# RVC-Project/obs-rvc

Hardware: AMD Instinct MI355X
Metric: audio frames/sec (10 ms hops of new input, 160 ms chunks @16 kHz) (higher is better)
Workload: dtype f32; 1 GPU; BASELINE configs[1]: 1 stream(s)/GPU, ContentVec v2-768 + RMVPE + NSF-HiFiGAN v2-48k, retrieval off, preset full; streams_per_gpu=1, streams_total=1, hip_graph=False

## Files before the change

obs_rvc_amd/csrc/conv_tile.hip.h:

```cpp
#pragma once
#include "igemm.hip.h"

namespace rvc {

#define COMMA_ ,
#ifndef RVC_CT_DBG
#define RVC_CT_DBG 0
#endif
template <int ACT, int MF, int NF>
__device__ __forceinline__ void conv_tile_store(const IgemmP &p, const PhaseD &ph, const float *resb, float *yb, const ColOut (&cols)[NF], int m_base, const f32x4 (&acc)[MF][NF])
{
    const float slope = p.slope, scale = p.scale;
    const long long cs = p.y_cs, rcs = p.res_cs;
#pragma unroll
    for (int mf = 0; mf < MF; mf++) {
        const int m0 = m_base + mf * 16;
        float bias_r[4];
#pragma unroll
        for (int r = 0; r < 4; r++) bias_r[r] = (p.bias && m0 + r < p.M) ? p.bias[ph.bias_off + m0 + r] : 0.f;
#pragma unroll
        for (int nf = 0; nf < NF; nf++) {
            if (cols[nf].yo < 0) continue;
            float rr[4] = {0.f, 0.f, 0.f, 0.f}, yo[4] = {0.f, 0.f, 0.f, 0.f};
            float *yc = yb + cols[nf].yo + (long long)(m0 + ph.y_c0) * cs;
            if (resb) {
                const float *rp = resb + cols[nf].ro + (long long)(p.res_nogroup ? m0 : m0 + ph.y_c0) * rcs;
#pragma unroll
                for (int r = 0; r < 4; r++) if (m0 + r < p.M) rr[r] = rp[r * rcs];
            }
            if (p.accumulate) {
#pragma unroll
                for (int r = 0; r < 4; r++) if (m0 + r < p.M) yo[r] = yc[r * cs];
            }
#pragma unroll
            for (int r = 0; r < 4; r++)
                if (m0 + r < p.M) yc[r * cs] = epi2_value<ACT>(acc[mf][nf][r], bias_r[r], rr[r], yo[r], slope, scale);
        }
    }
}

template <int WM, int WN, int MF, int NF, int KS>
__global__ __launch_bounds__(64 * WM * WN * KS) __attribute__((amdgpu_waves_per_eu(2))) void conv_tile_kernel(IgemmP p)
{
    static_assert(KS == 1 || KS == 2, "one or two K shares");
    constexpr int WPS = WM * WN, NT = 64 * WPS * KS;
    constexpr int BM = WM * MF * 16, BN = WN * NF * 16;
    constexpr int DA = MF == 1 ? 8 : 6;
    extern __shared__ __attribute__((aligned(16))) int s_mem[];
    const int item = p.items[2 * blockIdx.x];
    if (item < 0) return;
    RVC_KP(0);
    const int phase = item & 0xff, tm = (item >> 8) & 0xff, tn = item >> 16;
    const int b = p.items[2 * blockIdx.x + 1];
    const PhaseD ph = p.nphase == 1 ? p.ph0 : p.ph[phase];
    const int nchunks = ph.nchunks;
    const int lane = threadIdx.x & 63;
    const int wave = __builtin_amdgcn_readfirstlane((int)(threadIdx.x >> 6));
    const int kh = wave / WPS, w4 = wave % WPS;
    const int wm = w4 / WN, wn = w4 % WN;
    const int li = lane & 15, kq = lane >> 4;
    const int cin = ph.t_cin, rt = ph.t_rs, kw = ph.t_tab & 0xff, dil = ph.t_tab >> 8;
    const int rl = BN + (kw - 1) * dil;
    const int cs = cin + 8;
    const int G = cin >> 4;
    float *tmp = reinterpret_cast<float *>(s_mem);
    const int tmp_n = (cin * rt + 63) & ~63;
    float *fin = tmp + (tmp_n > WPS * MF * NF * 256 ? tmp_n : WPS * MF * NF * 256);
    {
        const float *xb = p.x + (long long)b * p.x_bs + ph.x_off;
        const int n0 = tn * BN + ph.t_dmin;
        const int total = cin * rt;
        const float inv_rt = 1.0f / (float)rt;
        for (int q = wave; q * 64 < total; q += WPS * KS) {
            const int e = q * 64 + lane;
            int row = (int)(((float)e + 0.5f) * inv_rt);
            const int col = e - row * rt;
            row = row < cin ? row : cin - 1;
            int gc = n0 + col;
            gc = gc < p.x_lo ? p.x_lo : (gc > p.x_lim ? p.x_lim : gc);
            __builtin_amdgcn_global_load_lds(xb + (long long)row * p.x_ld + gc, (__attribute__((address_space(3))) void *)(tmp + q * 64), 4, 0, 0);
        }
    }
    RVC_KP(1);
    const float *wrow[MF];
    const int mtiles = (p.M + 15) >> 4;
#pragma unroll
    for (int mf = 0; mf < MF; mf++) {
        int mt = (tm * WM + wm) * MF + mf;
        mt = mt < mtiles ? mt : mtiles - 1;
        wrow[mf] = p.w + ph.w_off + (long long)mt * nchunks * 256;
    }
    const int nloc = (nchunks - kh + KS - 1) / KS;
    const unsigned lane16 = (unsigned)lane * 16u;
    const float *wnext[MF];
#pragma unroll
    for (int mf = 0; mf < MF; mf++) wnext[mf] = wrow[mf] + (long long)(kh + DA * KS) * 256;
    f32x4 a_st[DA][MF];
#pragma unroll
    for (int s = 0; s < DA; s++) {
        const int cc = kh + (s < nloc ? s : nloc - 1) * KS;
#pragma unroll
        for (int mf = 0; mf < MF; mf++) a_st[s][mf] = *reinterpret_cast<const f32x4 *>(wrow[mf] + cc * 256 + lane * 4);
    }
    f32x4 acc[MF][NF];
#pragma unroll
    for (int mf = 0; mf < MF; mf++)
#pragma unroll
        for (int nf = 0; nf < NF; nf++) acc[mf][nf] = (f32x4){0.f, 0.f, 0.f, 0.f};
    const float pre_slope = p.pre_slope;
    RVC_KP(11);
    __syncthreads();
    {
        const int total = cin * rl;
        const float inv_cin = 1.0f / (float)cin;
        for (int e = threadIdx.x; e < total; e += NT) {
            const int col = (int)(((float)e + 0.5f) * inv_cin), ci = e - col * cin;
            const float v = tmp[ci * rt + col];
            fin[col * cs + ci] = fmaxf(v, v * pre_slope);
        }
    }
    __syncthreads();
    RVC_KP(2);
    const float *bl = fin + (wn * NF * 16 + li) * cs + kq * 4;
    const int last = nloc - 1;
    int g_b = 0, off_b = 0;
    const int wrap_b = dil * cs - 16 * G;
#define RVC_CT_ADV1() { g_b++; off_b += 16; if (g_b == G) { g_b = 0; off_b += wrap_b; } }
#define RVC_CT_ADV() { g_b += KS; off_b += 16 * KS; if (g_b >= G) { g_b -= G; off_b += wrap_b; } }
    if (kh) RVC_CT_ADV1()
    f32x4 bcur[NF];
#pragma unroll
    for (int nf = 0; nf < NF; nf++) bcur[nf] = *reinterpret_cast<const f32x4 *>(bl + off_b + nf * 16 * cs);
    RVC_CT_ADV()
    constexpr int T_ = MF * NF * 4;
#define RVC_CT_STEP(S, CC)                                                                              \
    {                                                                                                  \
        const int cc_ = (CC);                                                                          \
        const int ob_ = cc_ < last ? off_b : 0;                  \
        f32x4 bnx_[NF];                                                                                \
        _Pragma("unroll") for (int t = 0; t < T_; t++) {                                               \
            const int j = t / (NF * MF), nf = (t / MF) % NF, mf = t % MF;                              \
            if (!(RVC_CT_DBG & 8)) acc[mf][nf] = __builtin_amdgcn_mfma_f32_16x16x4f32(a_st[S][mf][j], bcur[nf][j], acc[mf][nf], 0, 0, 0); \
            else acc[mf][nf][0] += a_st[S][mf][j] * bcur[nf][j];                                       \
                                     \
            _Pragma("unroll") for (int r = t * NF / T_; r < (t + 1) * NF / T_; r++) {                  \
                if (!(RVC_CT_DBG & 2)) bnx_[r] = *reinterpret_cast<const f32x4 *>(bl + ob_ + r * 16 * cs); else bnx_[r] = bcur[r]; \
            }                                                                                          \
            __builtin_amdgcn_sched_barrier(0);                                                         \
        }                                                                                              \
         \
        if (!(RVC_CT_DBG & 1)) {                                                                       \
            _Pragma("unroll") for (int mf = 0; mf < MF; mf++) a_st[S][mf] = *reinterpret_cast<const f32x4 *>(reinterpret_cast<const char *>(wnext[mf]) + lane16); \
        }                                                                                              \
        __builtin_amdgcn_sched_barrier(0);                                                             \
        RVC_CT_ADV()                                                                                   \
        _Pragma("unroll") for (int mf = 0; mf < MF; mf++) wnext[mf] += KS * 256;       \
        _Pragma("unroll") for (int nf = 0; nf < NF; nf++) bcur[nf] = bnx_[nf];                         \
    }
    int c = 0;
    for (; c + DA <= nloc; c += DA) {
#pragma unroll
        for (int s = 0; s < DA; s++) RVC_CT_STEP(s, c + s)
    }
#pragma unroll
    for (int s = 0; s < DA; s++)
        if (c + s < nloc) RVC_CT_STEP(s, c + s)
#undef RVC_CT_STEP
#undef RVC_CT_ADV
#undef RVC_CT_ADV1
    RVC_KP(3);
    if (KS == 2) {
        f32x4 *red = reinterpret_cast<f32x4 *>(tmp) + (w4 * MF * NF) * 64 + lane;
        if (kh) {
#pragma unroll
            for (int mf = 0; mf < MF; mf++)
#pragma unroll
                for (int nf = 0; nf < NF; nf++) red[(mf * NF + nf) * 64] = acc[mf][nf];
        }
        __syncthreads();
        if (kh) return;
#pragma unroll
        for (int mf = 0; mf < MF; mf++)
#pragma unroll
            for (int nf = 0; nf < NF; nf++) { const f32x4 o = red[(mf * NF + nf) * 64]; acc[mf][nf][0] += o[0]; acc[mf][nf][1] += o[1]; acc[mf][nf][2] += o[2]; acc[mf][nf][3] += o[3]; }
    }
    const float *resb = p.res ? p.res + (long long)b * p.res_bs : nullptr;
    float *yb = p.y + (long long)b * p.y_bs + ph.y_off;
    const int act_sel = ph.act_p1 ? ph.act_p1 - 1 : p.act;
    ColOut cols[NF];
#pragma unroll
    for (int nf = 0; nf < NF; nf++) cols[nf] = col_locate(p, ph, tn * BN + (wn * NF + nf) * 16 + li);
    RVC_ACT_DISPATCH_SEL(act_sel, conv_tile_store<A_ COMMA_ MF COMMA_ NF>(p, ph, resb, yb, cols, ((tm * WM + wm) * MF) * 16 + kq * 4, acc);)
    RVC_KP(6);
}
#undef COMMA_

}
```

obs_rvc_amd/csrc/debug.hip:

```cpp
#include "engine_int.h"
#include "../../include/rvc_mi355x_debug.h"
#include <deque>

namespace {

struct DebugGeo {
    float *base = nullptr; long long g[8] = {0, 0, 0, 0, 0, 0, 0, 1};
    bool live() const { return base && g[0] > 0; }
    void upload(const float *h) const { if (live()) HIPCHK(hipMemcpy(base, h, (size_t)g[0] * 4, hipMemcpyHostToDevice)); }
    void download(float *h) const { if (live()) HIPCHK(hipMemcpy(h, base, (size_t)g[0] * 4, hipMemcpyDeviceToHost)); }
};
DebugGeo debug_geo1(const T1 &t)
{
    DebugGeo q; const size_t gd = t1_guard(t.ld);
    q.base = t.p - gd - t.halo; q.g[0] = (long long)t.B * t.bs + 2 * (long long)gd; q.g[1] = (long long)gd + t.halo; q.g[2] = t.C; q.g[3] = t.T; q.g[4] = t.ld; q.g[5] = t.bs; q.g[6] = t.ld;
    return q;
}
DebugGeo debug_geo2(const T2 &t)
{
    DebugGeo q; const size_t gd = t2_guard(t.ld);
    q.base = t.p - gd - t.ld - 1; q.g[0] = (long long)t.B * t.bs + 2 * (long long)gd; q.g[1] = (long long)gd + t.ld + 1; q.g[2] = t.C; q.g[3] = t.W; q.g[4] = t.ld; q.g[5] = t.bs; q.g[6] = t.cs; q.g[7] = t.H;
    return q;
}
DebugGeo debug_geo_flat(float *p, long long n, int C, int T) { DebugGeo q; q.base = p; q.g[0] = n; q.g[1] = 0; q.g[2] = C; q.g[3] = T; q.g[4] = T; q.g[5] = (long long)C * T; q.g[6] = T; return q; }
// ... 9 lines not shown
        try { for (auto &o : pl.ops.v) o(e->stream); } catch (...) { end_failed_capture(e->stream); throw; }
        HIPCHK(hipStreamEndCapture(e->stream, &g));
        const hipError_t ie = hipGraphInstantiate(&ge, g, nullptr, nullptr, 0);
        (void)hipGraphDestroy(g);
        HIPCHK(ie);
        hipError_t le = hipSuccess;
        for (int r = 0; r < reps && le == hipSuccess; r++) le = hipGraphLaunch(ge, e->stream);
        const hipError_t se = hipStreamSynchronize(e->stream);
        (void)hipGraphExecDestroy(ge);
        HIPCHK(le); HIPCHK(se);
    } else {
        for (int r = 0; r < reps; r++) for (auto &o : pl.ops.v) o(e->stream);
        HIPCHK(hipStreamSynchronize(e->stream));
    }
    HIPCHK(hipGetLastError());
}

struct DebugWeights {
    std::deque<ConvW> convs; std::vector<float *> raw;
    DebugWeights() = default;
    DebugWeights(const DebugWeights &) = delete;
    ConvW &conv(ConvW c) { convs.push_back(std::move(c)); return convs.back(); }
    float *dev(float *p) { raw.push_back(p); return p; }
    ~DebugWeights() { for (ConvW &c : convs) free_conv(c); for (float *p : raw) wfree(p); }
};

void fill_weights(std::vector<float> &w) { for (size_t i = 0; i < w.size(); i++) w[i] = (float)((i * 2654435761u) % 1000) / 1000.0f - 0.5f; }
void fill_input(std::vector<float> &x) { for (size_t i = 0; i < x.size(); i++) x[i] = (float)(((i * 40503u) ^ (i >> 3)) % 2001) / 1000.0f - 1.0f; }

}

extern "C" {

int rvc_debug_stamps(rvc_engine *e, char *buf, size_t cap)
{
    if (!e || !e->last_plan || !e->last_plan->d_stamps) return 0;
    Plan &pl = *e->last_plan;
    std::vector<unsigned long long> h(pl.stamp_names.size());
    if (hipMemcpy(h.data(), pl.d_stamps, h.size() * 8, hipMemcpyDeviceToHost) != hipSuccess) return 0;
    unsigned long long t0 = ~0ull; for (auto v : h) t0 = std::min(t0, v);
    std::string out;
    for (size_t i = 0; i < h.size(); i++) { char ln[96]; snprintf(ln, sizeof ln, "%s %.2f\n", pl.stamp_names[i].c_str(), (double)(h[i] - t0) / 100.0); out += ln; }
    if (out.size() + 1 > cap) return -1;
    memcpy(buf, out.c_str(), out.size() + 1);
    return (int)h.size();
}

#ifdef RVC_TUNING
double rvc_debug_conv_bench(rvc_engine *e, int M, int Cin, int KW, int dil, int N, int iters, int pre_act, int streams, int act)
{
    double us = -1.0;
    (void)guarded(e, [&]() {
        std::vector<float> w((size_t)M * Cin * KW), bias(M, 0.1f);
        fill_weights(w);
        const int Bb = streams > 0 ? streams : 1;
        Plan pl; pl.B = Bb;
        DebugWeights wts;
        ConvW &cw = wts.conv(prep_conv(w.data(), bias.data(), M, Cin, KW, 1));
        const int pad = (KW - 1) * dil / 2;
        T1 x = make_t1(pl.arena, Bb, Cin, N, (pad + 3) / 4 * 4), y = make_t1(pl.arena, Bb, M, N, 0);
        std::vector<float> hx((size_t)Cin * x.ld, 0.25f);
        for (int b = 0; b < Bb; b++) HIPCHK(hipMemcpy(x.p + (long long)b * x.bs - x.halo, hx.data(), hx.size() * 4, hipMemcpyHostToDevice));
        ConvOpts o; if (pre_act) { o.pre_act = ACT_LRELU; o.pre_slope = 0.1f; }
        o.act = act;
        add_conv1d(pl, cw, x, y, 1, pad, dil, o);
        run_ops(e, pl, 3, false);
        hipEvent_t a, b; HIPCHK(hipEventCreate(&a)); HIPCHK(hipEventCreate(&b));
        HIPCHK(hipEventRecord(a, e->stream));
        for (int i = 0; i < iters; i++) for (auto &op : pl.ops.v) op(e->stream);
        HIPCHK(hipEventRecord(b, e->stream));
        HIPCHK(hipStreamSynchronize(e->stream));
        float ms; HIPCHK(hipEventElapsedTime(&ms, a, b));
        us = ms * 1e3 / iters;
        (void)hipEventDestroy(a); (void)hipEventDestroy(b);
        return RVC_OK;
    });
    return us;
}

int rvc_debug_conv_probe(rvc_engine *e, int M, int Cin, int KW, int dil, int N, unsigned long long *out, size_t cap_waves, double *event_us, int *waves_per_wg)
{
    int nw = -1;
    (void)guarded(e, [&]() {
        std::vector<float> w((size_t)M * Cin * KW), bias(M, 0.1f);
        fill_weights(w);
        Plan pl; pl.B = 1;
        DebugWeights wts;
        ConvW &cw = wts.conv(prep_conv(w.data(), bias.data(), M, Cin, KW, 1));
        const int pad = (KW - 1) * dil / 2;
        T1 x = make_t1(pl.arena, 1, Cin, N, (pad + 3) / 4 * 4), y = make_t1(pl.arena, 1, M, N, 0);
        std::vector<float> hx((size_t)Cin * x.ld, 0.25f);
        HIPCHK(hipMemcpy(x.p - x.halo, hx.data(), hx.size() * 4, hipMemcpyHostToDevice));
        const size_t pbytes = (size_t)1 << 24;
        unsigned long long *d_probe = (unsigned long long *)pl.arena.alloc(pbytes);
        ConvOpts o; if (const char *a = tune_env("RVC_BENCH_ACT")) o.act = atoi(a);
        {
            struct Probing { Probing(unsigned long long *p) { g_kprobe = p; } ~Probing() { g_kprobe = nullptr; } } probing(d_probe);
            add_conv1d(pl, cw, x, y, 1, pad, dil, o);
        }
        run_ops(e, pl, 5, false);
        HIPCHK(hipMemset(d_probe, 0, pbytes));
        pl.profile = true; pl.prof_used = 0;
        run_ops(e, pl, 1, false);
        float t = 0.f; HIPCHK(hipEventElapsedTime(&t, pl.prof[0].a, pl.prof[0].b));
        if (event_us) *event_us = t * 1e3;
        nw = g_last_wgs * g_last_waves;
        if (waves_per_wg) *waves_per_wg = g_last_waves;
        if ((size_t)nw <= cap_waves && (size_t)nw * 128 <= pbytes) HIPCHK(hipMemcpy(out, d_probe, (size_t)nw * 128, hipMemcpyDeviceToHost));
        else nw = -2;
        return RVC_OK;
    });
    return nw;
}
#endif

double rvc_debug_ln_fold_check(rvc_engine *e, int M, int K, int N, float offset)
{
    double worst = -1.0;
    (void)guarded(e, [&]() {
        if (K % 16 != 0) throw ShapeError("K must be a multiple of 16");
        auto rnd = [](size_t i, unsigned salt) { return (float)((((i + 1) * 2654435761u) ^ (salt * 40503u) ^ (i >> 5)) % 2001) / 1000.0f - 1.0f; };
        std::vector<float> w1((size_t)M * K), b1(M), w2((size_t)K * M), b2(K), g(K), beta(K), hx((size_t)K * N), hz((size_t)M * N);
        for (size_t i = 0; i < w1.size(); i++) w1[i] = 0.5f * rnd(i, 1);
        for (size_t i = 0; i < w2.size(); i++) w2[i] = 0.5f * rnd(i, 2);
        for (int m = 0; m < M; m++) b1[m] = 0.1f * rnd(m, 3);
        for (int k = 0; k < K; k++) { b2[k] = 0.1f * rnd(k, 4); g[k] = 1.0f + 0.3f * rnd(k, 5); beta[k] = 0.2f * rnd(k, 6); }
        for (size_t i = 0; i < hx.size(); i++) hx[i] = 2.0f * rnd(i, 7) + offset;
        for (size_t i = 0; i < hz.size(); i++) hz[i] = rnd(i, 8);
        Plan pl; pl.B = 1;
        DebugWeights wts;
        float *wsum = nullptr;
        ConvW &c1 = wts.conv(ModelCV::fold_ln(w1.data(), b1.data(), M, K, g.data(), beta.data(), &wsum));
        wts.dev(wsum);
        ConvW &c2 = wts.conv(prep_conv(w2.data(), b2.data(), K, M, 1, 1));
        float *dg = wts.dev(upload_f(g)), *dbeta = wts.dev(upload_f(beta));
        T1 x = make_t1(pl.arena, 1, K, N, 0), y1 = make_t1(pl.arena, 1, M, N, 0), z = make_t1(pl.arena, 1, M, N, 0), y2 = make_t1(pl.arena, 1, K, N, 0);
        float *st = pl.arena.floats((size_t)2 * N + 16);
        for (int k = 0; k < K; k++) HIPCHK(hipMemcpy(x.p + (long long)k * x.ld, &hx[(size_t)k * N], (size_t)N * 4, hipMemcpyHostToDevice));
        for (int m = 0; m < M; m++) HIPCHK(hipMemcpy(z.p + (long long)m * z.ld, &hz[(size_t)m * N], (size_t)N * 4, hipMemcpyHostToDevice));
        { ConvOpts o; o.ln_wsum = wsum; o.ln_stats_out = st; o.ln_rows = K; add_conv1d(pl, c1, x, y1, 1, 0, 1, o); }
        { ConvOpts o; o.res = x.p; o.res_cs = x.ld; o.res_bs = x.bs; o.ln_stats_in = st; o.ln_g = dg; o.ln_b = dbeta; add_conv1d(pl, c2, z, y2, 1, 0, 1, o); }
        run_ops(e, pl, 1, false);
        std::vector<double> ln((size_t)K * N), mean(N), rstd(N);
        for (int n = 0; n < N; n++) {
            double s = 0; for (int k = 0; k < K; k++) s += hx[(size_t)k * N + n];
            const double mu = s / K; double q = 0;
            for (int k = 0; k < K; k++) { const double d = hx[(size_t)k * N + n] - mu; q += d * d; }
            mean[n] = mu; rstd[n] = 1.0 / std::sqrt(q / K + 1e-5);
            for (int k = 0; k < K; k++) ln[(size_t)k * N + n] = (hx[(size_t)k * N + n] - mu) * rstd[n] * g[k] + beta[k];
        }
        double err = 0.0;
        std::vector<float> row(N), hst((size_t)2 * N);
        {
            double ss = 0; std::vector<double> ref((size_t)M * N);
            for (int m = 0; m < M; m++) for (int n = 0; n < N; n++) {
                double a = b1[m]; for (int k = 0; k < K; k++) a += (double)w1[(size_t)m * K + k] * ln[(size_t)k * N + n];
                ref[(size_t)m * N + n] = a; ss += a * a;
            }
            const double rms1 = std::sqrt(ss / ((double)M * N)) + 1e-12;
            for (int m = 0; m < M; m++) {
                HIPCHK(hipMemcpy(row.data(), y1.p + (long long)m * y1.ld, (size_t)N * 4, hipMemcpyDeviceToHost));
                for (int n = 0; n < N; n++) err = std::max(err, std::fabs((double)row[n] - ref[(size_t)m * N + n]) / rms1);
            }
        }
        {
            double ss = 0; std::vector<double> ref((size_t)K * N);
            for (int k = 0; k < K; k++) for (int n = 0; n < N; n++) {
                double a = b2[k]; for (int m = 0; m < M; m++) a += (double)w2[(size_t)k * M + m] * hz[(size_t)m * N + n];
                a += ln[(size_t)k * N + n];
                ref[(size_t)k * N + n] = a; ss += a * a;
            }
            const double rms2 = std::sqrt(ss / ((double)K * N)) + 1e-12;
            for (int k = 0; k < K; k++) {
                HIPCHK(hipMemcpy(row.data(), y2.p + (long long)k * y2.ld, (size_t)N * 4, hipMemcpyDeviceToHost));
                for (int n = 0; n < N; n++) err = std::max(err, std::fabs((double)row[n] - ref[(size_t)k * N + n]) / rms2);
            }
        }
        HIPCHK(hipMemcpy(hst.data(), st, (size_t)2 * N * 4, hipMemcpyDeviceToHost));
        for (int n = 0; n < N; n++) {
            err = std::max(err, std::fabs((double)hst[2 * n] - mean[n]) / (std::fabs(mean[n]) + 1.0));
            err = std::max(err, std::fabs((double)hst[2 * n + 1] - rstd[n]) / rstd[n]);
// ... 349 lines not shown
```

obs_rvc_amd/csrc/igemm.hip.h:

```cpp
#pragma once
#include <hip/hip_runtime.h>
#include <stdint.h>

namespace rvc {

typedef float f32x4 __attribute__((ext_vector_type(4)));

enum Act { ACT_NONE = 0, ACT_RELU = 1, ACT_LRELU = 2, ACT_GELU = 3, ACT_TANH = 4, ACT_SIGMOID = 5 };

#ifdef RVC_FAST_GELU
__device__ __forceinline__ float erf_dev(float x)
{
    x = fminf(fmaxf(x, -4.f), 4.f);
    const float x2 = x * x;
    float p = -2.72614225801306e-10f;
    p = fmaf(p, x2, 2.77068142495902e-08f); p = fmaf(p, x2, -2.10102402082508e-06f); p = fmaf(p, x2, -5.69250639462346e-05f);
    p = fmaf(p, x2, -7.34990630326855e-04f); p = fmaf(p, x2, -2.95459980854025e-03f); p = fmaf(p, x2, -1.60960333262415e-02f);
    float q = -1.45660718464996e-05f;
    q = fmaf(q, x2, -2.13374055278905e-04f); q = fmaf(q, x2, -1.68282697438203e-03f); q = fmaf(q, x2, -7.37332916720468e-03f); q = fmaf(q, x2, -1.42647390514189e-02f);
    return x * p * __builtin_amdgcn_rcpf(q);
}
#else
__device__ __forceinline__ float erf_dev(float x) { return erff(x); }
#endif
__device__ __forceinline__ float gelu_dev(float v) { return 0.5f * v * (1.0f + erf_dev(v * 0.70710678118654752440f)); }

__device__ __forceinline__ float apply_act(float v, int act, float slope)
{
    switch (act) {
    case ACT_RELU: return v > 0.f ? v : 0.f;
    case ACT_LRELU: return v > 0.f ? v : v * slope;
    case ACT_GELU: return gelu_dev(v);
    case ACT_TANH: return tanhf(v);
    case ACT_SIGMOID: return 1.0f / (1.0f + expf(-v));
    default: return v;
    }
}

struct PhaseD {
    long long w_off;
    int x_off;
    int y_c0;
    int y_h0;
    int y_pos;
    int bias_off;
    int koff_off;
    int nchunks;
    int act_p1;
    int pad_;
    long long y_off;
    int t_tab;
    int t_cin;
    int t_rs;
    int t_dmin;
};

struct IgemmP {
    const float *x, *w, *bias, *res;
    float *y, *part;
    const int *koff;
    const PhaseD *ph;
    PhaseD ph0;
    int M, N, K;
    int NW;
    int x_hs, x_ws;
    int y_hm, y_ws;
    int OW;
    long long x_bs, y_bs, res_bs;
    int y_cs, res_cs;
    int y_rs, res_rs;
    int nphase, ksplit, chunks_per_split;
    int act; float slope; float scale; int accumulate;
    int pre_act; float pre_slope;
    int ntn, ntm;
    int koff_bias;
    int glu;
    int res_nogroup;
    unsigned long long *probe;
    int m_fast;
    int nbatch;
    int fold_n;
    int bf3;
    int lin_cs4;
    const float *ln_wsum;
    float *ln_stats_out;
    const float *ln_stats_in, *ln_g, *ln_bt;
    float ln_eps, ln_inv_rows;
    const int *items, *ttab;
    int x_ld, x_lo, x_lim, pad2_;
};

__device__ __forceinline__ void epilogue_store(const IgemmP &p, const PhaseD &ph, int b, int m, int n, float acc)
{
    if (m >= p.M || n >= p.N) return;
    if (p.fold_n) { b = n / p.fold_n; n -= b * p.fold_n; }
    int nh = 0, nw = n;
    if (p.y_hm) { nh = n / p.NW; nw = n - nh * p.NW; }
    const int ow = nw * p.y_ws + ph.y_pos, oh = nh * p.y_hm + ph.y_h0;
    if (ow < 0 || ow >= p.OW) return;
    const int ch = m + ph.y_c0;
    float v = acc;
    if (p.bias) v += p.bias[ph.bias_off + m];
    v = apply_act(v, p.act, p.slope);
    if (p.res) v += p.res[(long long)b * p.res_bs + (long long)(p.res_nogroup ? m : ch) * p.res_cs + (long long)oh * p.res_rs + ow];
    v *= p.scale;
    float *yp = p.y + (long long)b * p.y_bs + (long long)ch * p.y_cs + (long long)oh * p.y_rs + ow;
    if (p.accumulate) v += *yp;
    *yp = v;
}

__device__ __forceinline__ void glu_store(const IgemmP &p, const PhaseD &ph, int b, int m1, int n, float a1, float a2)
{
    if (m1 >= p.M || n >= p.N) return;
    if (p.fold_n) { b = n / p.fold_n; n -= b * p.fold_n; }
    const float ta = a1 + p.bias[ph.bias_off + m1], sa = a2 + p.bias[ph.bias_off + m1 + 2];
    const int ch = (m1 >> 4) * 8 + ((m1 & 15) >> 2) * 2 + (m1 & 1) + ph.y_c0;
    p.y[(long long)b * p.y_bs + (long long)ch * p.y_cs + n] = tanhf(ta) * (1.0f / (1.0f + expf(-sa)));
}

struct EpiPre { float bias, res, yold; };
__device__ __forceinline__ bool epi_locate(const IgemmP &p, const PhaseD &ph, int m, int n, int &ch, int &oh, int &ow)
{
    if (m >= p.M || n >= p.N) return false;
    int nh = 0, nw = n;
    if (p.y_hm) { nh = n / p.NW; nw = n - nh * p.NW; }
    ow = nw * p.y_ws + ph.y_pos; oh = nh * p.y_hm + ph.y_h0;
    if (ow < 0 || ow >= p.OW) return false;
    ch = m + ph.y_c0;
    return true;
}
__device__ __forceinline__ EpiPre epi_prefetch(const IgemmP &p, const PhaseD &ph, int b, int m, int n)
{
    EpiPre e = {0.f, 0.f, 0.f};
    int ch, oh, ow;
    if (!epi_locate(p, ph, m, n, ch, oh, ow)) return e;
    if (p.bias) e.bias = p.bias[ph.bias_off + m];
    if (p.res) e.res = p.res[(long long)b * p.res_bs + (long long)(p.res_nogroup ? m : ch) * p.res_cs + (long long)oh * p.res_rs + ow];
    if (p.accumulate) e.yold = p.y[(long long)b * p.y_bs + (long long)ch * p.y_cs + (long long)oh * p.y_rs + ow];
    return e;
}
__device__ __forceinline__ void epi_finish(const IgemmP &p, const PhaseD &ph, int b, int m, int n, float acc, const EpiPre &e)
{
    int ch, oh, ow;
    if (!epi_locate(p, ph, m, n, ch, oh, ow)) return;
    float v = apply_act(acc + e.bias, p.act, p.slope);
    v += e.res;
    v *= p.scale;
    v += e.yold;
    p.y[(long long)b * p.y_bs + (long long)ch * p.y_cs + (long long)oh * p.y_rs + ow] = v;
}

__device__ __forceinline__ void lds_only_barrier()
{
    __builtin_amdgcn_s_waitcnt(0xC07F);
    __builtin_amdgcn_s_barrier();
}

#ifdef RVC_KPROBE
#define RVC_KP(i) do { if (p.probe && (threadIdx.x & 63) == 0) p.probe[((size_t)((blockIdx.z * gridDim.y + blockIdx.y) * gridDim.x + blockIdx.x) * (blockDim.x >> 6) + (threadIdx.x >> 6)) * 16 + (i)] = wall_clock64(); } while (0)
#else
#define RVC_KP(i)
#endif
template <int MF, int NF, int D, int KS, bool PRE>
__global__ __launch_bounds__((KS > 1 ? KS : 4) * 64) void igemm_kernel(IgemmP p)
{
    constexpr int WAVES = KS > 1 ? KS : 4;
    RVC_KP(0);
    constexpr int NACC = (MF * NF == 1) ? 2 : 1;
    constexpr int TE = MF * NF * 256;
    constexpr int PE = (KS > 1) ? ((TE + WAVES * 64 - 1) / (WAVES * 64)) : 1;
    constexpr bool PF = (KS > 1) || (MF * NF <= 4);
    extern __shared__ __attribute__((aligned(16))) int s_koff[];
    const int lane = threadIdx.x & 63, wave = threadIdx.x >> 6;
    const int tile = KS > 1 ? (int)blockIdx.x : (int)blockIdx.x * 4 + wave;
    int z = blockIdx.y;
    const int ks = z % p.ksplit; z /= p.ksplit;
    const int phase = z % p.nphase;
    const int b = z / p.nphase;
    const PhaseD ph = p.nphase == 1 ? p.ph0 : p.ph[phase];
    const int nchunks = ph.nchunks;
    const int g0 = ks * p.chunks_per_split;
    int g1 = g0 + p.chunks_per_split;
    g1 = g1 < nchunks ? g1 : nchunks;
    const int gn = g1 - g0;
    {
        const int4 *src = reinterpret_cast<const int4 *>(p.koff + ph.koff_off + g0 * 16);
        int4 *dst = reinterpret_cast<int4 *>(s_koff);
        for (int i = threadIdx.x; i < gn * 4; i += WAVES * 64) dst[i] = src[i];
    }
    RVC_KP(8);
    int tn, tm;
    if (p.m_fast) { tm = tile % p.m_fast; tn = tile / p.m_fast; }
    else { tn = tile % p.ntn; tm = tile / p.ntn; }
    const bool live = tm < p.ntm && tn < p.ntn;
    const int li = lane & 15, kq = lane >> 4;

    EpiPre pre_w[(KS > 1 || !PF) ? 1 : MF][(KS > 1 || !PF) ? 1 : NF][4];
    EpiPre pre_r[PE];
    if (PF && live && p.ksplit == 1) {
        if (KS > 1) {
#pragma unroll
            for (int q = 0; q < PE; q++) {
                const int e = threadIdx.x + q * WAVES * 64;
                const int l = e & 63, r = (e >> 6) & 3, f = e >> 8, mf = f / NF, nf = f - mf * NF;
                pre_r[q] = (e < TE) ? epi_prefetch(p, ph, b, tm * 16 * MF + mf * 16 + (l >> 4) * 4 + r, tn * 16 * NF + nf * 16 + (l & 15)) : EpiPre{0.f, 0.f, 0.f};
            }
        } else {
#pragma unroll
            for (int mf = 0; mf < ((KS > 1 || !PF) ? 1 : MF); mf++)
#pragma unroll
                for (int nf = 0; nf < ((KS > 1 || !PF) ? 1 : NF); nf++)
#pragma unroll
                    for (int r = 0; r < 4; r++)
                        pre_w[mf][nf][r] = epi_prefetch(p, ph, b, tm * 16 * MF + mf * 16 + kq * 4 + r, tn * 16 * NF + nf * 16 + li);
        }
    }
    RVC_KP(9);
    int c0 = 0, nc = gn;
    if (KS > 1) {
        const int cpw = (gn + KS - 1) / KS;
        c0 = wave * cpw;
        int c1 = c0 + cpw;
        c1 = c1 < gn ? c1 : gn;
        nc = c1 > c0 ? c1 - c0 : 0;
    }

    const char *xb = reinterpret_cast<const char *>(p.x + (long long)b * p.x_bs + ph.x_off) - p.koff_bias;
    unsigned xo[NF];
#pragma unroll
    for (int nf = 0; nf < NF; nf++) {
        int n = tn * 16 * NF + nf * 16 + li;
        n = n < p.N ? n : p.N - 1;
        int nh = 0, nw = n;
        if (p.x_hs) { nh = n / p.NW; nw = n - nh * p.NW; }
        xo[nf] = (unsigned)(nh * p.x_hs + nw * p.x_ws) * 4u;
    }
    const float *wrow[MF];
    const int mtiles = (p.M + 15) >> 4;
#pragma unroll
    for (int mf = 0; mf < MF; mf++) {
        int mt = tm * MF + mf;
        mt = mt < mtiles ? mt : mtiles - 1;
        wrow[mf] = p.w + ph.w_off + ((long long)mt * nchunks + (g0 + c0)) * 256 + lane * 4;
    }
// ... 1397 lines not shown
```

obs_rvc_amd/csrc/plan.hip:

```cpp
#include "engine_int.h"
#include <chrono>

namespace rvc {

struct TestHook { const char *name; bool planner; };
static const TestHook kTestHooks[] = {
    {"RVC_FORCE_CFG", true}, {"RVC_CONV_TILE", true}, {"RVC_CONV_TILE_KS", true}, {"RVC_NO_LN_FUSE", false}, {"RVC_NO_CONV0_MULTI", false},
    {"RVC_KNN_NO_GEMM", false}, {"RVC_KNN_EXHAUSTIVE", false}, {"RVC_STAMPS", false}, {"RVC_SERIAL_BRANCHES", false}, {"RVC_NO_WN_COMPOSE", false},
    {"RVC_KNN_LOSE_TICKET", false}, {"RVC_FORCE_G2W", true}, {"RVC_F0_XCDS", false}, {"RVC_CONV32S", true}, {"RVC_CONV32S_TILE", true},
    {"RVC_G32L", true}, {"RVC_G32L_TALL", true}, {"RVC_G32L_TAB", true}, {"RVC_CONV32S_BUF", true}, {"RVC_FORCE_CHOICE", true},
    {"RVC_G32L_PANEL", true}, {"RVC_MEAN3", false}, {"RVC_RM_FUSE", false}, {"RVC_G2W_LN", false}, {"RVC_RELPOS_MFMA_MAX", false},
    {"RVC_ATTN_KERNEL", false}, {"RVC_RELPOS_KERNEL", false}, {"RVC_LN_KERNEL", false}, {"RVC_GRU_KERNEL", false}, {"RVC_CONV0_KERNEL", false},
    {"RVC_YIN_CV_ALL_CUS", false}
};
std::atomic<unsigned> g_opt_gen{0};
static std::mutex g_opt_mu;
static std::map<std::string, std::string> g_opts;
static bool is_test_hook(const char *name)
{
    for (const TestHook &h : kTestHooks) if (!strcmp(h.name, name)) return true;
    return false;
}
static const char *opt_lookup(const char *name)
{
    static thread_local std::string buf;
    std::lock_guard<std::mutex> lk(g_opt_mu);
    auto it = g_opts.find(name);
    if (it == g_opts.end()) return nullptr;
    buf = it->second;
    return buf.c_str();
}
#ifdef RVC_TUNING
const char *test_opt(const char *name) { const char *v = opt_lookup(name); return v ? v : getenv(name); }
const char *tune_env(const char *name) { const char *v = opt_lookup(name); return v ? v : getenv(name); }
#else
const char *test_opt(const char *name) { return opt_lookup(name); }
#endif
int test_opt_int(const char *name, int dflt) { const char *v = test_opt(name); return v ? atoi(v) : dflt; }

namespace {
struct WSlab { char *base; size_t size, used; long live; int dev, cls; };
std::mutex g_wslab_mu;
std::vector<WSlab> g_wslabs;
const size_t kWSlabBytes = (size_t)256 << 20, kPlanSlabBytes = (size_t)64 << 20;
void *wmalloc_cls(size_t bytes, int cls)
{
    bytes = (std::max<size_t>(bytes, 16) + 255) / 256 * 256;
    std::lock_guard<std::mutex> lk(g_wslab_mu);
    int dev = 0; HIPCHK(hipGetDevice(&dev));
    const size_t slab = cls ? kPlanSlabBytes : kWSlabBytes;
    if (bytes <= slab / 4) {
        for (size_t i = g_wslabs.size(); i-- > 0; ) {
            WSlab &b = g_wslabs[i];
            if (b.dev == dev && b.cls == cls && b.size == slab && b.used + bytes <= b.size) {
                void *r = b.base + b.used; b.used += bytes; b.live++;
                return r;
            }
        }
    }
    const size_t sz = bytes <= slab / 4 ? slab : bytes;
    void *c;
    HIPCHK(hipMalloc(&c, sz));
    g_wslabs.push_back(WSlab{(char *)c, sz, bytes, 1, dev, cls});
    return c;
}
}
void *wmalloc(size_t bytes) { return wmalloc_cls(bytes, 0); }
void *wmalloc_plan(size_t bytes) { return wmalloc_cls(bytes, 1); }
void wfree(void *p)
{
    if (!p) return;
    std::lock_guard<std::mutex> lk(g_wslab_mu);
    for (size_t i = 0; i < g_wslabs.size(); i++) {
        WSlab &b = g_wslabs[i];
        if ((char *)p >= b.base && (char *)p < b.base + b.size) {
            if (--b.live == 0) { (void)hipFree(b.base); g_wslabs.erase(g_wslabs.begin() + i); }
            return;
        }
    }
    (void)hipFree(p);
}
void wslab_info(int dev, int *count, size_t *bytes)
{
    std::lock_guard<std::mutex> lk(g_wslab_mu);
    *count = 0; *bytes = 0;
    for (const WSlab &b : g_wslabs) if (b.dev == dev) { (*count)++; *bytes += b.size; }
}

float *upload_f(const std::vector<float> &v, int cls)
{
    float *d = (float *)(cls ? wmalloc_plan(std::max<size_t>(v.size(), 4) * sizeof(float)) : wmalloc(std::max<size_t>(v.size(), 4) * sizeof(float)));
    if (!v.empty()) HIPCHK(hipMemcpy(d, v.data(), v.size() * sizeof(float), hipMemcpyHostToDevice));
    return d;
}
float *upload_f(const float *p, size_t n) { return upload_f(std::vector<float>(p, p + n)); }

// ... 184 lines not shown
    const int K = q.nchunks * 16;
    int cin = 1;
    for (int k = 0; k < K; k++) cin = std::max(cin, (int)std::floor((double)koff[q.koff_off + k] / p.x_ld + 0.5) + 1);
    if (cin % cblk != 0 || K % cin != 0) return false;
    const int KW = K / cin;
    if (KW > 255) return false;
    const int dmin = koff[q.koff_off];
    const int dil = KW > 1 ? koff[q.koff_off + 1] - koff[q.koff_off] : 1;
    if (dil < 1 || dil > 255 || dmin > 0 || dmin < p.x_lo) return false;
    for (int k = 0; k < K; k++) if (koff[q.koff_off + k] != (k / KW) * p.x_ld + dmin + (k % KW) * dil) return false;
    q.t_tab = KW | (dil << 8); q.t_cin = cin; q.t_dmin = dmin;
    return true;
}

static bool queue_conv_tile(GemmCall &c, IgemmP p, int B, const std::vector<PhaseD> &phv)
{
    const int mode = c.ch.kind ? 0 : test_opt_int("RVC_CONV_TILE", 1);
    if (!mode || p.fold_n || p.x_ld <= 0 || p.x_hs || p.x_ws != 1 || p.y_hm || p.lin_cs4 || p.glu || p.ln_wsum || p.ln_stats_in || p.ln_stats_out || p.part) return false;
    if (B > 4) return false;
    if (p.M > 128 && mode < 2) return false;
    const int kshares = test_opt_int("RVC_CONV_TILE_KS", 2);
    const int tc0 = p.M > 64 ? 0 : (p.M > 32 ? 1 : 2);
    const int BM = kTileBM[tc0], BN = kTileBN[tc0];
    const int ntm = (p.M + BM - 1) / BM, ntn = (p.N + BN - 1) / BN;
    if (ntm > 255 || ntn > 32767 || phv.size() > 255) return false;
    const long long nitems = (long long)ntm * ntn * (long long)phv.size() * B;
    if (mode < 2 && nitems < 3 * g_ncu / 2) return false;
    std::vector<PhaseD> phs(phv);
    std::vector<float> wnew;
    size_t lds_max = 0;
    const int mt = (p.M + 15) / 16;
    for (PhaseD &q : phs) {
        if (!decode_taps(q, c.koff, p, 16)) return false;
        const int KW = q.t_tab & 0xff, dil = q.t_tab >> 8, cin = q.t_cin;
        const int rl = BN + (KW - 1) * dil, rt = rl | 1, cs = cin + 8;
        q.t_rs = rt;
        if (q.nchunks < 2 || cin / 16 < kshares) return false;
        lds_max = std::max(lds_max, (std::max<size_t>(((size_t)cin * rt + 63) / 64 * 64, (size_t)kTileWF[tc0] * 256) + (size_t)rl * cs) * 4);
        std::vector<float> wold((size_t)mt * q.nchunks * 256);
        HIPCHK(hipMemcpy(wold.data(), p.w + q.w_off, wold.size() * 4, hipMemcpyDeviceToHost));
        const size_t base = wnew.size();
        wnew.resize(base + wold.size());
        const int G = cin / 16;
        for (int t = 0; t < mt; t++)
            for (int tap = 0; tap < KW; tap++)
                for (int g = 0; g < G; g++)
                    for (int l = 0; l < 64; l++)
                        for (int j = 0; j < 4; j++) {
                            const int k = (g * 16 + (l >> 4) * 4 + j) * KW + tap;
                            wnew[base + (((size_t)t * q.nchunks + tap * G + g) * 64 + l) * 4 + j] =
                                wold[(((size_t)t * q.nchunks + k / 16) * 64 + (((k % 16) / 4) << 4 | (l & 15))) * 4 + (k % 4)];
                        }
        q.w_off = (long long)base;
    }
    if (lds_max > 100 * 1024) return false;
    Plan &pl = c.pl;
    wnew.resize(wnew.size() + (size_t)16 * 2 * 256, 0.f);
    p.w = pl.arena.upload(wnew);
    struct It { int w, code, b; };
    std::vector<It> items;
    for (int bb = 0; bb < B; bb++)
        for (size_t f = 0; f < phs.size(); f++)
            for (int tm = 0; tm < ntm; tm++)
                for (int tn = 0; tn < ntn; tn++) items.push_back({phs[f].nchunks + 12, (int)f | (tm << 8) | (tn << 16), bb});
    std::stable_sort(items.begin(), items.end(), [](const It &a, const It &b) { return a.w > b.w; });
    const int nb = g_ncu;
    std::vector<std::vector<int>> bins(nb);
    {
        std::vector<std::pair<long long, int>> heap;
        for (int j = 0; j < nb; j++) heap.push_back({0, j});
        auto cmp = [](const std::pair<long long, int> &a, const std::pair<long long, int> &b) { return a > b; };
        std::make_heap(heap.begin(), heap.end(), cmp);
        for (size_t i = 0; i < items.size(); i++) {
            std::pop_heap(heap.begin(), heap.end(), cmp);
            auto &top = heap.back();
            bins[top.second].push_back((int)i); top.first += items[i].w;
            std::push_heap(heap.begin(), heap.end(), cmp);
        }
    }
    size_t rounds = 0;
    for (auto &bn : bins) rounds = std::max(rounds, bn.size());
    const bool xcd_bins = nb % 8 == 0 && !tune_env("RVC_NO_TILE_XCD");
    auto slot_bin = [&](int j) { return xcd_bins ? (j % 8) * (nb / 8) + j / 8 : j; };
    std::vector<int> order(rounds * nb * 2, -1);
    for (int j = 0; j < nb; j++) {
        const std::vector<int> &bn = bins[slot_bin(j)];
        for (size_t r = 0; r < bn.size(); r++) { order[(r * nb + j) * 2] = items[bn[r]].code; order[(r * nb + j) * 2 + 1] = items[bn[r]].b; }
    }
    p.items = pl.arena.upload(order);
    p.ttab = nullptr;
    set_phases(pl, p, phs);
    p.ntm = ntm; p.ntn = ntn; p.ksplit = 1; p.nbatch = B; p.m_fast = 0;
    const dim3 grid((unsigned)(order.size() / 2), 1u);
    char d[200];
    snprintf(d, sizeof d, "tile M=%d N=%d K=%d B=%d nph=%d tile=%dx%d items=%lld grid=%u lds=%zu pre=%d ksum=%.0f", p.M, p.N, p.K, B, p.nphase, BM, BN, nitems, grid.x, lds_max, (int)(p.pre_act != ACT_NONE), c.ksum);
    queue_gemm_launch(pl, d, 2.0 * p.M * (double)p.N * c.ksum * B, (int)nitems, 4, c.final_out, p,
                      [=](const IgemmP &q, hipEvent_t ea, hipEvent_t eb, hipStream_t s) { launch_conv_tile(tc0, kshares, q, grid, lds_max, s, ea, eb); });
    return true;
}

static bool queue_conv32s(GemmCall &c, IgemmP p, int B, const std::vector<PhaseD> &phv)
{
    if (c.ch.kind != 0 && c.ch.kind != 1) return false;
    const bool chosen = c.ch.kind == 1;
    const int mode = chosen ? 2 : test_opt_int("RVC_CONV32S", 1);
    if (!mode || p.fold_n || p.x_ld <= 0 || p.x_hs || p.x_ws != 1 || p.y_hm || p.y_ws != 1 || p.glu || p.ln_wsum || p.ln_stats_in || p.ln_stats_out || p.part || p.bf3 || c.pl.bf3) return false;
    if (mode < 2 && (B <= 4 || p.N < 200 || p.M < 32)) return false;
    for (const PhaseD &q : phv) if (q.act_p1 != 0 || q.y_off != 0 || q.y_pos != 0) return false;
    auto wgs_of = [&](int t) { return (long long)((p.M + kC32sBM[t] - 1) / kC32sBM[t]) * ((p.N + kC32sBN[t] - 1) / kC32sBN[t]) * (long long)phv.size() * B; };
    int tile = p.M <= 32 ? 0 : (p.M <= 64 ? 1 : 2);
    const int forced = chosen ? (c.ch.a & 3) : test_opt_int("RVC_CONV32S_TILE", -1);
    if (forced >= 0 && forced <= 2) tile = forced;
    if (mode < 2 && wgs_of(tile) < 2 * g_ncu) return false;
    const int BM = kC32sBM[tile], BN = kC32sBN[tile];
    const int ntm = (p.M + BM - 1) / BM, ntn = (p.N + BN - 1) / BN;
    if (phv.size() > 65535 || B > 65535) return false;
    std::vector<PhaseD> phs(phv);
    size_t lds_max = 0;
    int kw_max = 0;
    for (PhaseD &q : phs) {
        if (!decode_taps(q, c.koff, p, kC32sCB)) return false;
        const int KW = q.t_tab & 0xff, dil = q.t_tab >> 8;
        if ((KW - 1) * dil > 64) return false;
        q.t_rs = 0;
        lds_max = std::max(lds_max, (size_t)(BN + (KW - 1) * dil) * kC32sCS * 4);
        kw_max = std::max(kw_max, KW);
    }
    if (lds_max > 60 * 1024) return false;
    if (mode < 2 && kw_max <= 3 && p.M >= 64 && B >= 24) return false;
    const float *w0 = nullptr;
    for (PhaseD &q : phs) {
        const float *panel = c32s_panel(p.w + q.w_off, p.M, q.nchunks, q.t_cin, q.t_tab & 0xff);
        if (!w0) w0 = panel;
        q.w_off = panel - w0;
    }
    p.w = w0;
    p.koff = nullptr; p.items = nullptr; p.ttab = nullptr;
    set_phases(c.pl, p, phs);
    p.ntm = ntm; p.ntn = ntn; p.ksplit = 1; p.nbatch = B; p.m_fast = 0;
    p.pad2_ = tune_env("RVC_C32S_DBG") ? atoi(tune_env("RVC_C32S_DBG")) : 0;
    const int buf_opt = chosen ? ((c.ch.a & 4) ? 2 : 0) : test_opt_int("RVC_CONV32S_BUF", 1);
    const int ltile = tile | ((tile == 1 && (buf_opt == 2 || (buf_opt == 1 && B < 24))) ? 4 : 0);
    const dim3 grid((unsigned)(ntm * ntn), (unsigned)B, (unsigned)p.nphase);
    char d[200];
    snprintf(d, sizeof d, "c32s M=%d N=%d K=%d B=%d nph=%d tile=%dx%d%s grid=%ux%ux%u lds=%zu pre=%d ksum=%.0f", p.M, p.N, p.K, B, p.nphase, BM, BN, (ltile & 4) ? "b" : "", grid.x, grid.y, grid.z, lds_max, (int)(p.pre_act != ACT_NONE), c.ksum);
    queue_gemm_launch(c.pl, d, 2.0 * p.M * (double)p.N * c.ksum * B, (int)(grid.x * grid.y * grid.z), 4, c.final_out, p,
                      [=](const IgemmP &q, hipEvent_t ea, hipEvent_t eb, hipStream_t s) { launch_conv32s(ltile, q, grid, lds_max, s, ea, eb); });
    c.built = Choice{1, ltile, 0};
    return true;
}

static bool queue_bf3(GemmCall &c, IgemmP p, int B, const std::vector<PhaseD> &phv)
{
    const int nchunks = p.K / 16;
    if (!((p.bf3 || c.pl.bf3) && !p.glu && !c.ln_fold && B == 1 && p.x_hs == 0 && p.y_hm == 0 && p.M >= 128 && nchunks >= 2 && !p.accumulate &&
          (size_t)nchunks * 64 + 2 * 2 * 128 * 48 <= 60 * 1024 &&
          (long long)((p.M + 127) / 128) * ((p.N + 127) / 128) * p.nphase >= 250)) return false;
    const bool pre = p.pre_act != ACT_NONE;
    const bool lin = p.lin_cs4 != 0 && p.nphase == 1 && !pre;
    const int nblk = (p.M + 31) / 32;
    size_t tot = 0;
    std::vector<size_t> off(phv.size());
    for (size_t f = 0; f < phv.size(); f++) { off[f] = tot; tot += (size_t)nblk * phv[f].nchunks * 2048; }
    float *wsplit = (float *)wmalloc_plan(tot);
    for (size_t f = 0; f < phv.size(); f++) bf3_pack(p.w + phv[f].w_off, p.M, phv[f].nchunks, (char *)wsplit + off[f], nullptr);
    HIPCHK(hipDeviceSynchronize());
    c.pl.owned_dev.push_back(wsplit);
    std::vector<PhaseD> ph3(phv);
    for (size_t f = 0; f < ph3.size(); f++) ph3[f].w_off = (long long)(off[f] / 4);
    p.w = wsplit;
    set_phases(c.pl, p, ph3);
    p.ksplit = 1; p.chunks_per_split = nchunks;
    p.ntm = (p.M + 127) / 128; p.ntn = (p.N + 127) / 128;
    p.m_fast = p.fold_n ? 1 : 0;
    const dim3 grid((unsigned)(p.ntm * p.ntn), (unsigned)p.nphase);
    const size_t lds = (lin ? 0 : (size_t)nchunks * 64) + (size_t)2 * 2 * 128 * 48;
// ... 852 lines not shown
```

Measured before the change: 8082 frames/s.

## Pack per-tile phase descriptors into 128-byte item records and prefetch epilogue operands

Each conv-tile work item now carries its code, batch index and a full copy of its phase descriptor in one 128-byte aligned record. The kernel reads a single cache line per item instead of first reading the item code and then indexing the phase table, which removes a dependent load. Bias, residual and accumulate operands are also loaded by the k-share-0 waves before the main K loop instead of after it, so their global latency overlaps the MFMA work. In exchange the item buffer is larger and the prefetched epilogue values stay in registers across the loop, which may raise register pressure; the debug probe also gains a fused and residual mode.

Result: no change. 8114 frames/s, median of 3 (+0.4%).

```diff
diff --git a/obs_rvc_amd/csrc/conv_tile.hip.h b/obs_rvc_amd/csrc/conv_tile.hip.h
--- a/obs_rvc_amd/csrc/conv_tile.hip.h
+++ b/obs_rvc_amd/csrc/conv_tile.hip.h
@@ -7,34 +7,49 @@
 #ifndef RVC_CT_DBG
 #define RVC_CT_DBG 0
 #endif
+template <int MF, int NF> struct CtEpi { float bias[MF][4], rr[MF][NF][4], yo[MF][NF][4]; };
+template <int MF, int NF>
+__device__ __forceinline__ void conv_tile_epi_load(const IgemmP &p, const PhaseD &ph, const float *resb, const float *yb, const ColOut (&cols)[NF], int m_base, CtEpi<MF, NF> &e)
+{
+    const long long cs = p.y_cs, rcs = p.res_cs;
+#pragma unroll
+    for (int mf = 0; mf < MF; mf++) {
+        const int m0 = m_base + mf * 16;
+#pragma unroll
+        for (int r = 0; r < 4; r++) e.bias[mf][r] = (p.bias && m0 + r < p.M) ? p.bias[ph.bias_off + m0 + r] : 0.f;
+#pragma unroll
+        for (int nf = 0; nf < NF; nf++) {
+#pragma unroll
+            for (int r = 0; r < 4; r++) e.rr[mf][nf][r] = e.yo[mf][nf][r] = 0.f;
+            if (cols[nf].yo < 0) continue;
+            if (resb) {
+                const float *rp = resb + cols[nf].ro + (long long)(p.res_nogroup ? m0 : m0 + ph.y_c0) * rcs;
+#pragma unroll
+                for (int r = 0; r < 4; r++) if (m0 + r < p.M) e.rr[mf][nf][r] = rp[r * rcs];
+            }
+            if (p.accumulate) {
+                const float *yc = yb + cols[nf].yo + (long long)(m0 + ph.y_c0) * cs;
+#pragma unroll
+                for (int r = 0; r < 4; r++) if (m0 + r < p.M) e.yo[mf][nf][r] = yc[r * cs];
+            }
+        }
+    }
+}
 template <int ACT, int MF, int NF>
-__device__ __forceinline__ void conv_tile_store(const IgemmP &p, const PhaseD &ph, const float *resb, float *yb, const ColOut (&cols)[NF], int m_base, const f32x4 (&acc)[MF][NF])
+__device__ __forceinline__ void conv_tile_store(const IgemmP &p, const PhaseD &ph, float *yb, const ColOut (&cols)[NF], int m_base, const f32x4 (&acc)[MF][NF], const CtEpi<MF, NF> &e)
 {
     const float slope = p.slope, scale = p.scale;
-    const long long cs = p.y_cs, rcs = p.res_cs;
+    const long long cs = p.y_cs;
 #pragma unroll
     for (int mf = 0; mf < MF; mf++) {
         const int m0 = m_base + mf * 16;
-        float bias_r[4];
-#pragma unroll
-        for (int r = 0; r < 4; r++) bias_r[r] = (p.bias && m0 + r < p.M) ? p.bias[ph.bias_off + m0 + r] : 0.f;
 #pragma unroll
         for (int nf = 0; nf < NF; nf++) {
             if (cols[nf].yo < 0) continue;
-            float rr[4] = {0.f, 0.f, 0.f, 0.f}, yo[4] = {0.f, 0.f, 0.f, 0.f};
             float *yc = yb + cols[nf].yo + (long long)(m0 + ph.y_c0) * cs;
-            if (resb) {
-                const float *rp = resb + cols[nf].ro + (long long)(p.res_nogroup ? m0 : m0 + ph.y_c0) * rcs;
-#pragma unroll
-                for (int r = 0; r < 4; r++) if (m0 + r < p.M) rr[r] = rp[r * rcs];
-            }
-            if (p.accumulate) {
-#pragma unroll
-                for (int r = 0; r < 4; r++) if (m0 + r < p.M) yo[r] = yc[r * cs];
-            }
 #pragma unroll
             for (int r = 0; r < 4; r++)
-                if (m0 + r < p.M) yc[r * cs] = epi2_value<ACT>(acc[mf][nf][r], bias_r[r], rr[r], yo[r], slope, scale);
+                if (m0 + r < p.M) yc[r * cs] = epi2_value<ACT>(acc[mf][nf][r], e.bias[mf][r], e.rr[mf][nf][r], e.yo[mf][nf][r], slope, scale);
         }
     }
 }
@@ -47,13 +62,25 @@
     constexpr int BM = WM * MF * 16, BN = WN * NF * 16;
     constexpr int DA = MF == 1 ? 8 : 6;
     extern __shared__ __attribute__((aligned(16))) int s_mem[];
-    const int item = p.items[2 * blockIdx.x];
-    if (item < 0) return;
-    RVC_KP(0);
-    const int phase = item & 0xff, tm = (item >> 8) & 0xff, tn = item >> 16;
-    const int b = p.items[2 * blockIdx.x + 1];
-    const PhaseD ph = p.nphase == 1 ? p.ph0 : p.ph[phase];
+    int item, b;
+    PhaseD ph;
+    if (p.ct_opts & 1) {
+        const CtItem rec = reinterpret_cast<const CtItem *>(p.items)[blockIdx.x];
+        item = rec.code; b = rec.b; ph = rec.ph;
+        if (item < 0) return;
+        RVC_KP(0);
+    } else {
+        item = p.items[2 * blockIdx.x];
+        if (item < 0) return;
+        RVC_KP(0);
+        b = p.items[2 * blockIdx.x + 1];
+        ph = p.nphase == 1 ? p.ph0 : p.ph[item & 0xff];
+    }
+    const int tm = (item >> 8) & 0xff, tn = item >> 16;
     const int nchunks = ph.nchunks;
+    RVC_KP_ARRIVED(nchunks);
+    RVC_KP(8);
+    RVC_KP_VAL(15, (item & 0xff) + 1);
     const int lane = threadIdx.x & 63;
     const int wave = __builtin_amdgcn_readfirstlane((int)(threadIdx.x >> 6));
     const int kh = wave / WPS, w4 = wave % WPS;
@@ -82,6 +109,17 @@
         }
     }
     RVC_KP(1);
+    const float *resb = p.res ? p.res + (long long)b * p.res_bs : nullptr;
+    float *yb = p.y + (long long)b * p.y_bs + ph.y_off;
+    const int m_base = ((tm * WM + wm) * MF) * 16 + kq * 4;
+    const bool epi_ahead = (p.ct_opts & 2) != 0;
+    ColOut cols[NF];
+    CtEpi<MF, NF> epi;
+    if (epi_ahead && kh == 0) {
+#pragma unroll
+        for (int nf = 0; nf < NF; nf++) cols[nf] = col_locate(p, ph, tn * BN + (wn * NF + nf) * 16 + li);
+        conv_tile_epi_load<MF, NF>(p, ph, resb, yb, cols, m_base, epi);
+    }
     const float *wrow[MF];
     const int mtiles = (p.M + 15) >> 4;
 #pragma unroll
@@ -110,6 +148,7 @@
     const float pre_slope = p.pre_slope;
     RVC_KP(11);
     __syncthreads();
+    RVC_KP(9);
     {
         const int total = cin * rl;
         const float inv_cin = 1.0f / (float)cin;
@@ -184,13 +223,16 @@
 #pragma unroll
             for (int nf = 0; nf < NF; nf++) { const f32x4 o = red[(mf * NF + nf) * 64]; acc[mf][nf][0] += o[0]; acc[mf][nf][1] += o[1]; acc[mf][nf][2] += o[2]; acc[mf][nf][3] += o[3]; }
     }
-    const float *resb = p.res ? p.res + (long long)b * p.res_bs : nullptr;
-    float *yb = p.y + (long long)b * p.y_bs + ph.y_off;
+    RVC_KP(4);
     const int act_sel = ph.act_p1 ? ph.act_p1 - 1 : p.act;
-    ColOut cols[NF];
-#pragma unroll
-    for (int nf = 0; nf < NF; nf++) cols[nf] = col_locate(p, ph, tn * BN + (wn * NF + nf) * 16 + li);
-    RVC_ACT_DISPATCH_SEL(act_sel, conv_tile_store<A_ COMMA_ MF COMMA_ NF>(p, ph, resb, yb, cols, ((tm * WM + wm) * MF) * 16 + kq * 4, acc);)
+    if (!epi_ahead) {
+#pragma unroll
+        for (int nf = 0; nf < NF; nf++) cols[nf] = col_locate(p, ph, tn * BN + (wn * NF + nf) * 16 + li);
+        conv_tile_epi_load<MF, NF>(p, ph, resb, yb, cols, m_base, epi);
+    }
+    RVC_KP_ARRIVED(epi.bias[MF - 1][3]); RVC_KP_ARRIVED(epi.rr[MF - 1][NF - 1][3]); RVC_KP_ARRIVED(epi.yo[MF - 1][NF - 1][3]);
+    RVC_KP(5);
+    RVC_ACT_DISPATCH_SEL(act_sel, conv_tile_store<A_ COMMA_ MF COMMA_ NF>(p, ph, yb, cols, m_base, acc, epi);)
     RVC_KP(6);
 }
 #undef COMMA_
diff --git a/obs_rvc_amd/csrc/debug.hip b/obs_rvc_amd/csrc/debug.hip
--- a/obs_rvc_amd/csrc/debug.hip
+++ b/obs_rvc_amd/csrc/debug.hip
@@ -115,21 +115,35 @@
 {
     int nw = -1;
     (void)guarded(e, [&]() {
-        std::vector<float> w((size_t)M * Cin * KW), bias(M, 0.1f);
-        fill_weights(w);
+        const bool fusedp = tune_env("RVC_PROBE_FUSED") && atoi(tune_env("RVC_PROBE_FUSED")), withres = tune_env("RVC_PROBE_RES") && atoi(tune_env("RVC_PROBE_RES"));
+        const int kws[3] = {3, 7, 11}, nconv = fusedp ? 3 : 1;
         Plan pl; pl.B = 1;
         DebugWeights wts;
-        ConvW &cw = wts.conv(prep_conv(w.data(), bias.data(), M, Cin, KW, 1));
-        const int pad = (KW - 1) * dil / 2;
-        T1 x = make_t1(pl.arena, 1, Cin, N, (pad + 3) / 4 * 4), y = make_t1(pl.arena, 1, M, N, 0);
+        std::vector<ConvW *> cws;
+        int pad_max = 0;
+        for (int j = 0; j < nconv; j++) {
+            const int kw = fusedp ? kws[j] : KW;
+            std::vector<float> w((size_t)M * Cin * kw), bias(M, 0.1f);
+            fill_weights(w);
+            cws.push_back(&wts.conv(prep_conv(w.data(), bias.data(), M, Cin, kw, 1)));
+            pad_max = std::max(pad_max, (kw - 1) * dil / 2);
+        }
+        if (fusedp) merge_convs(cws);
+        T1 x = make_t1(pl.arena, 1, Cin, N, (pad_max + 3) / 4 * 4), y = make_t1(pl.arena, 1, nconv * M, N, 0), r = make_t1(pl.arena, 1, M, N, 0);
         std::vector<float> hx((size_t)Cin * x.ld, 0.25f);
         HIPCHK(hipMemcpy(x.p - x.halo, hx.data(), hx.size() * 4, hipMemcpyHostToDevice));
         const size_t pbytes = (size_t)1 << 24;
         unsigned long long *d_probe = (unsigned long long *)pl.arena.alloc(pbytes);
         ConvOpts o; if (const char *a = tune_env("RVC_BENCH_ACT")) o.act = atoi(a);
+        if (withres) { o.res = r.p; o.res_cs = r.ld; o.res_bs = r.bs; }
         {
             struct Probing { Probing(unsigned long long *p) { g_kprobe = p; } ~Probing() { g_kprobe = nullptr; } } probing(d_probe);
-            add_conv1d(pl, cw, x, y, 1, pad, dil, o);
+            if (fusedp) {
+                std::vector<const ConvW *> cc(cws.begin(), cws.end());
+                std::vector<int> pads, dils;
+                for (int j = 0; j < nconv; j++) { pads.push_back((kws[j] - 1) * dil / 2); dils.push_back(dil); }
+                add_conv1d_multi(pl, cc, x, false, y, pads, dils, o, false);
+            } else add_conv1d(pl, *cws[0], x, y, 1, (KW - 1) * dil / 2, dil, o);
         }
         run_ops(e, pl, 5, false);
         HIPCHK(hipMemset(d_probe, 0, pbytes));
diff --git a/obs_rvc_amd/csrc/igemm.hip.h b/obs_rvc_amd/csrc/igemm.hip.h
--- a/obs_rvc_amd/csrc/igemm.hip.h
+++ b/obs_rvc_amd/csrc/igemm.hip.h
@@ -88,7 +88,11 @@
     float ln_eps, ln_inv_rows;
     const int *items, *ttab;
     int x_ld, x_lo, x_lim, pad2_;
+    int ct_opts;
 };
+
+struct alignas(128) CtItem { int code, b; PhaseD ph; };
+static_assert(sizeof(CtItem) == 128, "one CtItem = one 128-byte line");
 
 __device__ __forceinline__ void epilogue_store(const IgemmP &p, const PhaseD &ph, int b, int m, int n, float acc)
 {
@@ -158,8 +162,12 @@
 
 #ifdef RVC_KPROBE
 #define RVC_KP(i) do { if (p.probe && (threadIdx.x & 63) == 0) p.probe[((size_t)((blockIdx.z * gridDim.y + blockIdx.y) * gridDim.x + blockIdx.x) * (blockDim.x >> 6) + (threadIdx.x >> 6)) * 16 + (i)] = wall_clock64(); } while (0)
+#define RVC_KP_VAL(i, v) do { if (p.probe && (threadIdx.x & 63) == 0) p.probe[((size_t)((blockIdx.z * gridDim.y + blockIdx.y) * gridDim.x + blockIdx.x) * (blockDim.x >> 6) + (threadIdx.x >> 6)) * 16 + (i)] = (unsigned long long)(v); } while (0)
+#define RVC_KP_ARRIVED(v) asm volatile("" :: "v"(v))
 #else
 #define RVC_KP(i)
+#define RVC_KP_VAL(i, v)
+#define RVC_KP_ARRIVED(v)
 #endif
 template <int MF, int NF, int D, int KS, bool PRE>
 __global__ __launch_bounds__((KS > 1 ? KS : 4) * 64) void igemm_kernel(IgemmP p)
diff --git a/obs_rvc_amd/csrc/plan.hip b/obs_rvc_amd/csrc/plan.hip
--- a/obs_rvc_amd/csrc/plan.hip
+++ b/obs_rvc_amd/csrc/plan.hip
@@ -11,7 +11,7 @@
     {"RVC_G32L", true}, {"RVC_G32L_TALL", true}, {"RVC_G32L_TAB", true}, {"RVC_CONV32S_BUF", true}, {"RVC_FORCE_CHOICE", true},
     {"RVC_G32L_PANEL", true}, {"RVC_MEAN3", false}, {"RVC_RM_FUSE", false}, {"RVC_G2W_LN", false}, {"RVC_RELPOS_MFMA_MAX", false},
     {"RVC_ATTN_KERNEL", false}, {"RVC_RELPOS_KERNEL", false}, {"RVC_LN_KERNEL", false}, {"RVC_GRU_KERNEL", false}, {"RVC_CONV0_KERNEL", false},
-    {"RVC_YIN_CV_ALL_CUS", false}
+    {"RVC_YIN_CV_ALL_CUS", false}, {"RVC_CT_KARG", false}, {"RVC_CT_EPI_AHEAD", false}
 };
 std::atomic<unsigned> g_opt_gen{0};
 static std::mutex g_opt_mu;
@@ -362,16 +362,29 @@
     for (auto &bn : bins) rounds = std::max(rounds, bn.size());
     const bool xcd_bins = nb % 8 == 0 && !tune_env("RVC_NO_TILE_XCD");
     auto slot_bin = [&](int j) { return xcd_bins ? (j % 8) * (nb / 8) + j / 8 : j; };
-    std::vector<int> order(rounds * nb * 2, -1);
-    for (int j = 0; j < nb; j++) {
-        const std::vector<int> &bn = bins[slot_bin(j)];
-        for (size_t r = 0; r < bn.size(); r++) { order[(r * nb + j) * 2] = items[bn[r]].code; order[(r * nb + j) * 2 + 1] = items[bn[r]].b; }
-    }
-    p.items = pl.arena.upload(order);
+    const bool wide = test_opt_int("RVC_CT_KARG", 1) != 0;
+    p.ct_opts = (wide ? 1 : 0) | (test_opt_int("RVC_CT_EPI_AHEAD", 1) != 0 ? 2 : 0);
+    const size_t nslots = rounds * nb;
+    if (wide) {
+        std::vector<CtItem> recs(nslots);
+        for (CtItem &r : recs) { memset(&r, 0, sizeof r); r.code = -1; }
+        for (int j = 0; j < nb; j++) {
+            const std::vector<int> &bn = bins[slot_bin(j)];
+            for (size_t r = 0; r < bn.size(); r++) { CtItem &t = recs[r * nb + j]; t.code = items[bn[r]].code; t.b = items[bn[r]].b; t.ph = phs[t.code & 0xff]; }
+        }
+        p.items = reinterpret_cast<const int *>(pl.arena.upload(recs));
+    } else {
+        std::vector<int> order(nslots * 2, -1);
+        for (int j = 0; j < nb; j++) {
+            const std::vector<int> &bn = bins[slot_bin(j)];
+            for (size_t r = 0; r < bn.size(); r++) { order[(r * nb + j) * 2] = items[bn[r]].code; order[(r * nb + j) * 2 + 1] = items[bn[r]].b; }
+        }
+        p.items = pl.arena.upload(order);
+    }
     p.ttab = nullptr;
     set_phases(pl, p, phs);
     p.ntm = ntm; p.ntn = ntn; p.ksplit = 1; p.nbatch = B; p.m_fast = 0;
-    const dim3 grid((unsigned)(order.size() / 2), 1u);
+    const dim3 grid((unsigned)nslots, 1u);
     char d[200];
     snprintf(d, sizeof d, "tile M=%d N=%d K=%d B=%d nph=%d tile=%dx%d items=%lld grid=%u lds=%zu pre=%d ksum=%.0f", p.M, p.N, p.K, B, p.nphase, BM, BN, nitems, grid.x, lds_max, (int)(p.pre_act != ACT_NONE), c.ksum);
     queue_gemm_launch(pl, d, 2.0 * p.M * (double)p.N * c.ksum * B, (int)nitems, 4, c.final_out, p,
```
